# KevynUtopia/Frequency-Aware-Inverse-Consistent-OCTA-Super-Resolution

Hardware: AMD Instinct MI355X
Metric: train-step images/sec (G+D fwd+bwd) on 256x256 OCTA (higher is better)
Workload: dtype f32 (tensors and accumulators fp32; the convolutions' operands enter the matrix cores as f16x2 pairs: hi = f16(x 2^k), lo = f16(x 2^k - hi), k from the tensor's largest magnitude; 3 v_mfma_f32_32x32x16_f16 per product) on every map >= 24 wide with >= 16 channels; narrow maps, 1-channel stems / head

## Files before the change

### frequency-aware-inverse-consistent-octa-super-resolution_amd/csrc/igemm_bf16x3.hip

```cpp
#include "common.h"
#include "igemm_geom.h"
#include "pack_bodies.h"
#include "split16.h"
#include <cstdlib>
#include <cstdint>
#include <type_traits>

#ifndef SP_NCW8
#define SP_NCW8 0
#endif
#ifndef SP_MIN_W
#define SP_MIN_W 24
#endif
#ifndef SP_CDMA
#define SP_CDMA 0
#endif
#ifndef SP_SPLIT_BELOW
#define SP_SPLIT_BELOW 128
#endif
#ifndef SP_WIDE
#define SP_WIDE 1
#endif
#ifndef SP_PROD_FIRST
#define SP_PROD_FIRST 0
// ... 34 lines not shown

#ifndef SP_EPI_FAST
#define SP_EPI_FAST 1
#endif
#ifndef SP_ABLATE
#define SP_ABLATE 0
#endif

constexpr int SP_MT = 64;
static thread_local bool g_conv_residual_live = false;
constexpr int SP_NPI = 6;

__device__ __forceinline__ int reflect_idx_s(int i, int n) {
    i = i < 0 ? -i : i;
    return i >= n ? 2 * n - 2 - i : i;
}

__device__ __forceinline__ void ds_read_v8(bf16x8& dst, unsigned addr) { asm volatile("ds_read_b128 %0, %1" : "=v"(dst) : "v"(addr)); }

template <int I, int N, class F>
__device__ __forceinline__ void static_for_sp(F&& f) {
    if constexpr (I < N) {
        f(std::integral_constant<int, I>{});
        static_for_sp<I + 1, N>(f);
    }
}

template <int MI, int NI>
__device__ __forceinline__ void wait_all(bf16x8 (&a)[MI][2], bf16x8 (&b)[NI][2]) {
    if constexpr (MI == 2 && NI == 2)
        asm volatile("s_waitcnt lgkmcnt(0)" : "+v"(a[0][0]), "+v"(a[0][1]), "+v"(a[1][0]), "+v"(a[1][1]), "+v"(b[0][0]), "+v"(b[0][1]), "+v"(b[1][0]), "+v"(b[1][1]));
    else if constexpr (MI == 2 && NI == 1)
        asm volatile("s_waitcnt lgkmcnt(0)" : "+v"(a[0][0]), "+v"(a[0][1]), "+v"(a[1][0]), "+v"(a[1][1]), "+v"(b[0][0]), "+v"(b[0][1]));
    else if constexpr (MI == 1 && NI == 2)
        asm volatile("s_waitcnt lgkmcnt(0)" : "+v"(a[0][0]), "+v"(a[0][1]), "+v"(b[0][0]), "+v"(b[0][1]), "+v"(b[1][0]), "+v"(b[1][1]));
    else
        asm volatile("s_waitcnt lgkmcnt(0)" : "+v"(a[0][0]), "+v"(a[0][1]), "+v"(b[0][0]), "+v"(b[0][1]));
}

template <int MI, int NI>
__device__ __forceinline__ void wait_keep_next(bf16x8 (&a)[MI][2], bf16x8 (&b)[NI][2]) {
    if constexpr (MI == 2 && NI == 2)
        asm volatile("s_waitcnt lgkmcnt(8)" : "+v"(a[0][0]), "+v"(a[0][1]), "+v"(a[1][0]), "+v"(a[1][1]), "+v"(b[0][0]), "+v"(b[0][1]), "+v"(b[1][0]), "+v"(b[1][1]));
    else if constexpr (MI == 2 && NI == 1)
        asm volatile("s_waitcnt lgkmcnt(6)" : "+v"(a[0][0]), "+v"(a[0][1]), "+v"(a[1][0]), "+v"(a[1][1]), "+v"(b[0][0]), "+v"(b[0][1]));
    else if constexpr (MI == 1 && NI == 2)
        asm volatile("s_waitcnt lgkmcnt(6)" : "+v"(a[0][0]), "+v"(a[0][1]), "+v"(b[0][0]), "+v"(b[0][1]), "+v"(b[1][0]), "+v"(b[1][1]));
    else
        asm volatile("s_waitcnt lgkmcnt(4)" : "+v"(a[0][0]), "+v"(a[0][1]), "+v"(b[0][0]), "+v"(b[0][1]));
}

template <bool F16>
__global__ __launch_bounds__(256) void split_pack_kernel(const float* __restrict__ w, unsigned short* __restrict__ wp, const SplitGeom g) {
    split_pack_block<F16>(w, wp, g, blockIdx.x, gridDim.x);
}
__global__ __launch_bounds__(256) void split_absmax_kernel(const float* __restrict__ w, float* __restrict__ wp, const SplitGeom g) {
    __shared__ unsigned red[4];
    split_absmax_block(w, wp, g, (int)blockIdx.x, red);
}

template <int NI, int SI, bool QUAD, int NCW = 4, bool F16 = false>
__global__ __launch_bounds__(64 * (NCW + 4)) void igemm_bf16x3_kernel(const float* __restrict__ x, const __bf16* __restrict__ wp,
                                                           const float* __restrict__ bias, float* __restrict__ y, const SplitGeom g,
                                                           const int ksplit, const int wide, const unsigned* __restrict__ x_slot,
                                                           const unsigned* __restrict__ w_slot, const float* __restrict__ res) {
    constexpr int MI = 2, TH = NCW * NI, NT = 256, NPI = SP_NPI;
    extern __shared__ __attribute__((aligned(16))) char smem[];
    const int tid = threadIdx.x, lane = tid & 63, wave = tid >> 6;
    SPTRACE0(tid == 0, 8);
    const int l31 = lane & 31, lh = lane >> 5;
    const bool producer = (SP_PROD_FIRST && NCW == 4) ? wave < 4 : wave >= NCW;
    const int wn = NCW == 4 ? wave & 3 : (wave >= NCW ? wave - NCW : wave), stid = tid & 255;
    const int ph = blockIdx.z / ksplit, ks = blockIdx.z - ph * ksplit;
    const int GH = g.gh[ph], GW = g.gw[ph];
    const int tiles_x = (GW + 31) >> 5, tiles_y = (GH + TH - 1) / TH;
    const int tiles = tiles_x * tiles_y;
    const long total_tiles = (long)g.N * tiles;
    if ((long)blockIdx.x >= total_tiles) return;
#if SP_STAGGER
    for (int i = (int)((blockIdx.x + blockIdx.y + blockIdx.z) & 7); i > 0; --i) __builtin_amdgcn_s_sleep(SP_STAGGER);
#endif
    const int t0 = g.t0[ph], T = g.t0[ph + 1] - t0, TG = g.tg[ph];
    const int ntg = (T + TG - 1) / TG;
    const int PH = (TH - 1) * SI + g.span_y[ph] + 1, PW = 31 * SI + g.span_x[ph] + 1, PHW = PH * PW;
    const int ngroups = (g.C + 15) >> 4;
    const int gps = (ngroups + ksplit - 1) / ksplit;
    const int g0 = ks * gps;
    const int g1 = (g0 + gps) < ngroups ? (g0 + gps) : ngroups;
    if (g0 >= g1) return;
    const int m0 = blockIdx.y * SP_MT;
    const int IH = g.IH, IW = g.IW;
    const long chw = (long)IH * IW;
    const unsigned a_bytes = (unsigned)TG * 2048u;
    const unsigned p_bytes = (unsigned)(2 * PHW) * 16u;
    const unsigned A_base = 0, P_base = 4u * a_bytes, S_base = P_base + 4u * p_bytes;
    auto tile_coords = [&](long tl, int& n, int& ty, int& tx) {
        n = (int)((unsigned)tl / (unsigned)tiles);
        const int rt = (int)((unsigned)tl - (unsigned)n * (unsigned)tiles);
        ty = (int)((unsigned)rt / (unsigned)tiles_x);
        tx = rt - ty * tiles_x;
    };

    if (producer) {
        if constexpr (SP_PRIO != 0) __builtin_amdgcn_s_setprio(SP_PRIO);
        constexpr unsigned OOB = 0x80000000u;
        const unsigned cstep = 4u * (unsigned)chw;
        const float* xin = x;
        float sx = 1.f;
        constexpr int NSI = QUAD ? 2 : NPI;
        unsigned poff[NSI];
        float pv[NSI][8];
        constexpr int NQI = QUAD ? 2 : 1;
        unsigned qoff[NQI];
        f32x4s qv[NQI][8];
        const int qx0 = (-g.ox0[ph]) & 3;
        const bool cover = QUAD && !g.reflect;
        const int qs = cover && qx0 ? qx0 - 4 : qx0;
        const int nq = QUAD ? (cover ? (PW - qs + 3) >> 2 : (PW - qx0) >> 2) : 0;
        const int ns = cover ? 0 : PW - 4 * nq;
        const int nqi = 2 * PH * nq, nitems = 2 * PH * ns;
        int s_pos[NSI], q_pos[NQI];
        int s_slot[NSI], q_slot[NQI];
        {
            const float inv_ns = 1.0f / (float)(ns > 0 ? ns : 1), inv_nq = 1.0f / (float)(nq > 0 ? nq : 1);
#pragma unroll
            for (int i = 0; i < NSI; ++i) {
                const int it = stid + NT * i;
                s_pos[i] = -1;
                s_slot[i] = 0;
                if (it < nitems) {
                    const int h = it >= PH * ns ? 1 : 0;
                    const int r = it - h * PH * ns;
                    const int py = (int)(((float)r + 0.5f) * inv_ns);
                    const int sx = r - py * ns;
                    const int px = sx < qx0 ? sx : sx + 4 * nq;
                    s_pos[i] = py | ((px + 4) << 8) | (h << 16);
                    s_slot[i] = h * PHW + py * PW + px;
                }
            }
#pragma unroll
            for (int i = 0; i < NQI; ++i) {
                const int it = stid + NT * i;
                q_pos[i] = -1;
                q_slot[i] = 0;
                if (QUAD && it < nqi) {
                    const int h = it >= PH * nq ? 1 : 0;
                    const int r = it - h * PH * nq;
                    const int py = (int)(((float)r + 0.5f) * inv_nq);
                    const int px = qs + 4 * (r - py * nq);
                    q_pos[i] = py | ((px + 4) << 8) | (h << 16);
                    q_slot[i] = h * PHW + py * PW + px;
                }
            }
        }
        if constexpr ((SP_ABLATE & 2) != 0) {
            for (int i = 0; i < NSI; ++i)
                for (int j = 0; j < 8; ++j) pv[i][j] = (float)(tid + i + j);
            for (int i = 0; i < NQI; ++i)
                for (int j = 0; j < 8; ++j) qv[i][j] = f32x4s{(float)tid, (float)i, (float)j, 1.f};
        }
        auto compute_poff = [&](long tl) {
            int n, ty, tx;
            tile_coords(tl, n, ty, tx);
            const int y_base = ty * TH * SI + g.oy0[ph], x_base = tx * 32 * SI + g.ox0[ph];
            xin = x + (long)n * g.C * chw;
            auto off_of = [&](int pos) -> unsigned {
                if (pos < 0) return OOB;
                int iy = y_base + (pos & 0xff), ix = x_base + ((pos >> 8) & 0xff) - 4;
                if (g.reflect) {
                    iy = reflect_idx_s(iy, IH);
                    ix = reflect_idx_s(ix, IW);
                }
                if ((unsigned)iy < (unsigned)IH && (unsigned)ix < (unsigned)IW) return 4u * (unsigned)(8 * (pos >> 16) * (int)chw + iy * IW + ix);
                return OOB;
            };
#pragma unroll
            for (int i = 0; i < NSI; ++i) poff[i] = off_of(s_pos[i]);
#pragma unroll
            for (int i = 0; i < NQI; ++i) qoff[i] = off_of(q_pos[i]);
        };
        auto load_patch = [&](int grp) {
            if constexpr ((SP_ABLATE & 2) != 0) return;
            const long bytes = (long)(g.C - grp * 16) * chw * 4;
            const auto srd = __builtin_amdgcn_make_buffer_rsrc(const_cast<float*>(xin + (long)grp * 16 * chw), 0,
                                                               (int)(bytes < 0x7ffffff0L ? bytes : 0x7ffffff0L), 0x00020000);
            if constexpr (QUAD) {
#pragma unroll
                for (int i = 0; i < NQI; ++i)
                    if (NT * i < nqi) {
#pragma unroll
                        for (int j = 0; j < 8; ++j)
                            qv[i][j] = __builtin_bit_cast(f32x4s, __builtin_amdgcn_raw_buffer_load_b128(srd, qoff[i] + j * cstep, 0, 0));
                    }
            }
#pragma unroll
            for (int i = 0; i < NSI; ++i)
                if (NT * i < nitems) {
#pragma unroll
                    for (int j = 0; j < 8; ++j)
                        pv[i][j] = __builtin_bit_cast(float, __builtin_amdgcn_raw_buffer_load_b32(srd, poff[i] + j * cstep, 0, 0));
                }
        };
        auto store_patch = [&](int buf, auto&& hook) {
            if constexpr ((SP_ABLATE & 4) != 0) return;
            char* hi_p = smem + P_base + (buf * 2 + 0) * p_bytes;
            char* lo_p = smem + P_base + (buf * 2 + 1) * p_bytes;
            if constexpr (QUAD) {
#pragma unroll
                for (int i = 0; i < NQI; ++i) {
                    if (NT * i < nqi) {
                        const bool qok = q_pos[i] >= 0;
                        const int px0 = ((q_pos[i] >> 8) & 0xff) - 4;
#pragma unroll
                        for (int kp = 0; kp < 2; ++kp) {
                            unsigned hd[2][4], ld[2][4];
                            if constexpr (F16) {
#pragma unroll
                                for (int k = 0; k < 2; ++k) {
#pragma unroll
                                    for (int c2 = 0; c2 < 4; ++c2) {
                                        split_pair_scaled<true>(qv[i][2 * c2][2 * kp + k], qv[i][2 * c2 + 1][2 * kp + k], sx, hd[k][c2], ld[k][c2]);
                                        if (c2 & 1) hook();
                                    }
                                }
                            } else {
                            f32x2s lo[8];
#pragma unroll
                            for (int k = 0; k < 2; ++k)
#pragma unroll
                                for (int c2 = 0; c2 < 4; ++c2)
                                    hd[k][c2] = cvt_pair<F16>(qv[i][2 * c2][2 * kp + k], qv[i][2 * c2 + 1][2 * kp + k]);
                            hook();
#pragma unroll
                            for (int c = 0; c < 8; ++c) {
                                const unsigned d0 = hd[0][c >> 1], d1 = hd[1][c >> 1];
                                const f32x2s hf = {(c & 1) ? half_hi_f32<F16>(d0) : half_lo_f32<F16>(d0), (c & 1) ? half_hi_f32<F16>(d1) : half_lo_f32<F16>(d1)};
                                lo[c] = f32x2s{qv[i][c][2 * kp], qv[i][c][2 * kp + 1]} - hf;
                                if ((c & 3) == 3) hook();
                            }
#pragma unroll
                            for (int k = 0; k < 2; ++k)
#pragma unroll
                                for (int c2 = 0; c2 < 4; ++c2)
                                    ld[k][c2] = cvt_pair<F16>(lo[2 * c2][k], lo[2 * c2 + 1][k]);
                            }
#pragma unroll
                            for (int k = 0; k < 2; ++k) {
                                if (qok && (unsigned)(px0 + 2 * kp + k) < (unsigned)PW) {
                                    *reinterpret_cast<u32x4s*>(hi_p + (q_slot[i] + 2 * kp + k) * 16) = u32x4s{hd[k][0], hd[k][1], hd[k][2], hd[k][3]};
                                    *reinterpret_cast<u32x4s*>(lo_p + (q_slot[i] + 2 * kp + k) * 16) = u32x4s{ld[k][0], ld[k][1], ld[k][2], ld[k][3]};
                                }
                                hook();
                            }
                        }
                    }
                }
            }
#pragma unroll
            for (int i = 0; i < NSI; ++i) {
                if (s_pos[i] >= 0) {
                    u32x4s hv, lv;
#pragma unroll
                    for (int j = 0; j < 4; ++j) {
                        unsigned h, l;
                        split_pair_scaled<F16>(pv[i][2 * j], pv[i][2 * j + 1], sx, h, l);
                        hv[j] = h;
                        lv[j] = l;
                    }
                    *reinterpret_cast<u32x4s*>(hi_p + s_slot[i] * 16) = hv;
                    *reinterpret_cast<u32x4s*>(lo_p + s_slot[i] * 16) = lv;
                }
            }
        };
        const int wnu = __builtin_amdgcn_readfirstlane(wn);
        const char* const wbase = reinterpret_cast<const char*>(wp + g.pack_off[ph] + (long)m0 * 8);
        const long w_row = (long)g.Mpad * 16, w_plane = g.plane_stride * 2;
        const unsigned lane16 = (unsigned)lane * 16u;
        const char* d_src = wbase;
        char* d_dst = smem;
        int d_r = 0, d_rows = 0, d_rows2 = 0;
        auto begin_A = [&](int grp, int tgi, int abuf) {
            const int tb = tgi * TG;
            int nt = T - tb;
            nt = nt < TG ? nt : TG;
            d_rows = nt * 2;
            d_rows2 = ((SP_ABLATE & 1) || SP_CDMA) ? 0 : 2 * d_rows;
            d_r = wnu;
            d_src = wbase + ((long)grp * T + tb) * 2 * w_row;
            d_dst = smem + A_base + (abuf * 2) * a_bytes;
        };
        auto next_row = [&]() {
            if (d_r < d_rows2) {
                const int plane = d_r >= d_rows ? 1 : 0;
                const int rr = d_r - plane * d_rows;
                __builtin_amdgcn_global_load_lds((const __attribute__((address_space(1))) void*)(d_src + plane * w_plane + rr * w_row + lane16),
                                                 (__attribute__((address_space(3))) void*)(d_dst + plane * a_bytes + rr * 1024), 16, 0, 0);
                d_r += 4;
            }
            __builtin_amdgcn_sched_barrier(0);
        };
        auto rest_of_A = [&]() {
            while (d_r < d_rows2) next_row();
        };

        long tile_l = blockIdx.x;
        int grp_l = g0;
        bool valid_l = true;
        auto advance_l = [&]() {
            if (++grp_l >= g1) {
                grp_l = g0;
                tile_l += gridDim.x;
                valid_l = tile_l < total_tiles;
                if (valid_l) compute_poff(tile_l);
            }
        };
        int npl_full = 0;
        if constexpr ((SP_ABLATE & 2) == 0) {
            for (int i = 0; i < NQI; ++i) npl_full += (QUAD && NT * i < nqi) ? 8 : 0;
            for (int i = 0; i < NSI; ++i) npl_full += NT * i < nitems ? 8 : 0;
        }
        auto barrier_keep = [&](int n) {
            switch (n) {
                case 0: asm volatile("s_waitcnt vmcnt(0) lgkmcnt(0)\n\ts_barrier" ::: "memory"); break;
                case 8: asm volatile("s_waitcnt vmcnt(8) lgkmcnt(0)\n\ts_barrier" ::: "memory"); break;
                case 16: asm volatile("s_waitcnt vmcnt(16) lgkmcnt(0)\n\ts_barrier" ::: "memory"); break;
                case 24: asm volatile("s_waitcnt vmcnt(24) lgkmcnt(0)\n\ts_barrier" ::: "memory"); break;
                case 32: asm volatile("s_waitcnt vmcnt(32) lgkmcnt(0)\n\ts_barrier" ::: "memory"); break;
                case 40: asm volatile("s_waitcnt vmcnt(40) lgkmcnt(0)\n\ts_barrier" ::: "memory"); break;
                case 48: asm volatile("s_waitcnt vmcnt(48) lgkmcnt(0)\n\ts_barrier" ::: "memory"); break;
                default: asm volatile("s_waitcnt vmcnt(0) lgkmcnt(0)\n\ts_barrier" ::: "memory"); break;
            }
        };
        auto no_hook = [&]() {};

        SPTRACE0(tid == ((SP_PROD_FIRST && NCW == 4) ? 0 : 64 * NCW), 12);
        compute_poff(tile_l);
        load_patch(grp_l);
        SPTRACE0(tid == ((SP_PROD_FIRST && NCW == 4) ? 0 : 64 * NCW), 13);
        advance_l();
        begin_A(g0, 0, 0);
        if constexpr (SP_CDMA != 0) d_rows2 = (SP_ABLATE & 1) ? 0 : 2 * d_rows;
        rest_of_A();
        SPTRACE0(tid == ((SP_PROD_FIRST && NCW == 4) ? 0 : 64 * NCW), 14);
        if constexpr (F16) sx = f16x2_scale(absmax_read(x_slot));
        store_patch(0, no_hook);
        int in_flight = 0;
        if (valid_l) {
            load_patch(grp_l);
            advance_l();
        }
        SPTRACE0(tid == ((SP_PROD_FIRST && NCW == 4) ? 0 : 64 * NCW), 9);
        barrier_keep(0);
        SPTRACE0(tid == ((SP_PROD_FIRST && NCW == 4) ? 0 : 64 * NCW), 10);
        long tile = blockIdx.x;
        int slab = 0, pcount = 0;
        while (true) {
            const long next_tile = tile + gridDim.x;
            const bool has_next = next_tile < total_tiles;
            for (int grp = g0; grp < g1; ++grp, ++pcount) {
                const int pbuf = pcount & 1;
                const bool last_grp = grp + 1 >= g1;
                const bool more_patch = !last_grp || has_next;
                for (int tgi = 0; tgi < ntg; ++tgi, ++slab) {
                    const int abuf = slab & 1;
                    SPTRACE(tid == ((SP_PROD_FIRST && NCW == 4) ? 0 : 64 * NCW), 3072, slab, 0);
                    in_flight = 0;
                    const bool swap_patch = tgi == ntg - 1 && more_patch;
                    d_rows2 = 0;
                    if (tgi + 1 < ntg) begin_A(grp, tgi + 1, abuf ^ 1);
                    else if (!last_grp) begin_A(grp + 1, 0, abuf ^ 1);
                    else if (has_next) begin_A(g0, 0, abuf ^ 1);
                    if (swap_patch) store_patch(pbuf ^ 1, next_row);
                    SPTRACE(tid == ((SP_PROD_FIRST && NCW == 4) ? 0 : 64 * NCW), 1024, slab, 0);
                    rest_of_A();
                    SPTRACE(tid == ((SP_PROD_FIRST && NCW == 4) ? 0 : 64 * NCW), 1024, slab, 1);
                    if (swap_patch && valid_l) {
                        load_patch(grp_l);
                        advance_l();
                        in_flight = npl_full;
                    }
                    SPTRACE(tid == ((SP_PROD_FIRST && NCW == 4) ? 0 : 64 * NCW), 1024, slab, 2);
                    barrier_keep(in_flight);
                    SPTRACE(tid == ((SP_PROD_FIRST && NCW == 4) ? 0 : 64 * NCW), 1024, slab, 3);
                }
            }
            if (!has_next) break;
            tile = next_tile;
        }
        return;
    }

    int tapv = 0;
    if (lane < T) {
        const int tp = g.taps[t0 + lane];
        tapv = (tp & 0xff) * PW + ((tp >> 8) & 0xff);
    }
    f32x16 acc[MI][NI];
#pragma unroll
    for (int mi = 0; mi < MI; ++mi)
#pragma unroll
        for (int ni = 0; ni < NI; ++ni)
#pragma unroll
            for (int r = 0; r < 16; ++r) acc[mi][ni][r] = 0.f;
    const unsigned lds0 = (unsigned)(unsigned long)(__attribute__((address_space(3))) char*)smem;
    const unsigned a_lane = (unsigned)(lh * 64 + l31) * 16u;
    const unsigned b_lane = (unsigned)((lh * PH + (wn * NI) * SI) * PW + l31 * SI) * 16u;
    const unsigned b_row = (unsigned)(SI * PW) * 16u;

    const int wnu_c = __builtin_amdgcn_readfirstlane(wn);
    const char* const wbase_c = reinterpret_cast<const char*>(wp + g.pack_off[ph] + (long)m0 * 8);
    const long w_row_c = (long)g.Mpad * 16, w_plane_c = g.plane_stride * 2;
    const unsigned lane16_c = (unsigned)lane * 16u;
    const char* c_src = wbase_c;
    char* c_dst = smem;
    int c_r = 0, c_rows = 0, c_rows2 = 0;
    auto c_begin = [&](int grp, int tgi, int abuf) {
        const int tb2 = tgi * TG;
        int nt2 = T - tb2;
        nt2 = nt2 < TG ? nt2 : TG;
        c_rows = nt2 * 2;
        c_rows2 = 2 * c_rows;
        c_r = wnu_c;
        c_src = wbase_c + ((long)grp * T + tb2) * 2 * w_row_c;
        c_dst = smem + A_base + (abuf * 2) * a_bytes;
    };
    auto c_next_row = [&]() {
        if (c_r < c_rows2) {
            const int plane = c_r >= c_rows ? 1 : 0;
            const int rr = c_r - plane * c_rows;
            __builtin_amdgcn_global_load_lds((const __attribute__((address_space(1))) void*)(c_src + plane * w_plane_c + rr * w_row_c + lane16_c),
                                             (__attribute__((address_space(3))) void*)(c_dst + plane * a_bytes + rr * 1024), 16, 0, 0);
            c_r += 4;
        }
    };

    float inv = 1.f;
    if constexpr (F16) inv = f16x2_inv_scale(absmax_read(x_slot)) * f16x2_inv_scale(split_w_absmax(w_slot));
    long tile = blockIdx.x;
    asm volatile("s_barrier" ::: "memory");
    int slab = 0, pcount = 0;
    while (true) {
        const long next_tile = tile + gridDim.x;
        const bool has_next = next_tile < total_tiles;
        for (int grp = g0; grp < g1; ++grp, ++pcount) {
            const int pbuf = pcount & 1;
            for (int tgi = 0; tgi < ntg; ++tgi, ++slab) {
                const int abuf = slab & 1;
                const int tb = tgi * TG;
                int nt = T - tb;
                nt = nt < TG ? nt : TG;
                const unsigned Ah = lds0 + A_base + (abuf * 2 + 0) * a_bytes + a_lane, Al = Ah + a_bytes;
                const unsigned Ph = lds0 + P_base + (pbuf * 2 + 0) * p_bytes + b_lane, Pl = Ph + p_bytes;
                bf16x8 a0[MI][2], b0[NI][2], a1[MI][2], b1[NI][2];
                auto rd_all = [&](bf16x8 (&a)[MI][2], bf16x8 (&b)[NI][2], int tl) {
                    const unsigned ao = (unsigned)tl * 2048u;
                    const unsigned bo = 16u * (unsigned)__builtin_amdgcn_readlane(tapv, (tb + tl) & 63);
#pragma unroll
                    for (int mi = 0; mi < MI; ++mi) {
                        ds_read_v8(a[mi][0], Ah + ao + mi * 512u);
                        ds_read_v8(a[mi][1], Al + ao + mi * 512u);
                    }
#pragma unroll
                    for (int ni = 0; ni < NI; ++ni) {
                        ds_read_v8(b[ni][0], Ph + bo + ni * b_row);
                        ds_read_v8(b[ni][1], Pl + bo + ni * b_row);
                    }
                };
                auto step = [&](bf16x8 (&a)[MI][2], bf16x8 (&b)[NI][2], bf16x8 (&an)[MI][2], bf16x8 (&bn)[NI][2], int tl_next) {
                    const unsigned ao = (unsigned)tl_next * 2048u;
                    const unsigned bo = 16u * (unsigned)__builtin_amdgcn_readlane(tapv, (tb + tl_next) & 63);
                    wait_all<MI, NI>(a, b);
                    static_for_sp<0, 3 * MI * NI>([&](auto jc) {
                        constexpr int j = decltype(jc)::value;
                        constexpr int term = j / (MI * NI), t = j % (MI * NI), mi = t / NI, ni = t % NI;
                        if constexpr ((SP_ABLATE & 8) != 0) {
                            if constexpr (j == 0) acc[0][0][0] += (float)a[0][0][0] + (float)a[MI - 1][1][0] + (float)b[0][0][0] + (float)b[NI - 1][1][0];
                        } else {
                            mfma16<F16>(a[mi][term == 0 ? 1 : 0], b[ni][term == 1 ? 1 : 0], acc[mi][ni]);
                        }
                        if constexpr (j < 2 * MI) ds_read_v8(an[j / 2][j % 2], (j % 2 ? Al : Ah) + ao + (j / 2) * 512u);
                        else if constexpr (j < 2 * (MI + NI)) ds_read_v8(bn[(j - 2 * MI) / 2][(j - 2 * MI) % 2], ((j - 2 * MI) % 2 ? Pl : Ph) + bo + ((j - 2 * MI) / 2) * b_row);
                        __builtin_amdgcn_sched_barrier(0);
                    });
                };
                SPTRACE(tid == ((SP_PROD_FIRST && NCW == 4) ? 256 : 0), 2048, slab, 0);
                if constexpr (SP_CDMA != 0) {
                    c_rows2 = 0;
                    const bool last_grp_c = grp + 1 >= g1;
                    if (tgi + 1 < ntg) c_begin(grp, tgi + 1, abuf ^ 1);
                    else if (!last_grp_c) c_begin(grp + 1, 0, abuf ^ 1);
// ... 112 lines not shown
                        for (int rr = 0; rr < 16; ++rr) S[((rr & 3) + 8 * (rr >> 2) + 4 * lh) * 32 + l31] = acc[mi][ni][rr];
#pragma unroll
                        for (int i = 0; i < 4; ++i) {
                            f32x4s v = *reinterpret_cast<const f32x4s*>(S + (prow + 8 * i) * 32 + 4 * pq);
                            const int dm = mi * 32 + 8 * i;
                            if (ok && (full_m || m0 + prow + dm < g.M) && ((SP_ABLATE & 16) == 0 || v[0] == 123.456f)) {
                                if (res) v += *reinterpret_cast<const f32x4s*>(rimg + (o0 + (unsigned)dm * ohw));
                                *reinterpret_cast<f32x4s*>(yimg + (o0 + (unsigned)dm * ohw)) = v;
                            }
                        }
                    }
                }
            } else
#pragma unroll
            for (int ni = 0; ni < NI; ++ni) {
                const int ao = cty * TH + wn * NI + ni;
                if (ao < GH && bo < GW) {
                    const unsigned o0 = (unsigned)mrow0 * ohw + (unsigned)((ao * g.SO + g.py[ph]) * g.OW + (bo * g.SO + g.px[ph]));
                    if (SP_EPI_FAST && (SP_ABLATE & 16) == 0 && full_m) {
                        auto emit = [&](auto atomic_c, auto res_c) {
                            constexpr bool AT = decltype(atomic_c)::value, RS = decltype(res_c)::value;
#pragma unroll
                            for (int mi = 0; mi < MI; ++mi) {
                                float r[16];
                                if constexpr (RS) {
#pragma unroll
                                    for (int rr = 0; rr < 16; ++rr) r[rr] = rimg[o0 + (unsigned)(mi * 32 + (rr & 3) + 8 * (rr >> 2)) * ohw];
                                }
#pragma unroll
                                for (int rr = 0; rr < 16; ++rr) {
                                    float* const p = yimg + (o0 + (unsigned)(mi * 32 + (rr & 3) + 8 * (rr >> 2)) * ohw);
                                    float v = acc[mi][ni][rr];
                                    if constexpr (RS) v += r[rr];
                                    if constexpr (AT) atomicAdd(p, v);
                                    else *p = v;
                                }
                            }
                        };
                        const bool use_res = res && ks == 0;
                        if (ksplit > 1) {
                            if (use_res) emit(std::true_type{}, std::true_type{});
                            else emit(std::true_type{}, std::false_type{});
                        } else {
                            if (use_res) emit(std::false_type{}, std::true_type{});
                            else emit(std::false_type{}, std::false_type{});
                        }
                    } else
#pragma unroll
                    for (int mi = 0; mi < MI; ++mi) {
#pragma unroll
                        for (int rr = 0; rr < 16; ++rr) {
                            const int dm = mi * 32 + (rr & 3) + 8 * (rr >> 2);
                            if ((full_m || mrow0 + dm < g.M) && ((SP_ABLATE & 16) == 0 || acc[mi][ni][rr] == 123.456f)) {
                                float* const p = yimg + (o0 + (unsigned)dm * ohw);
                                const float rv = (res && ks == 0) ? rimg[o0 + (unsigned)dm * ohw] : 0.f;
                                if (ksplit > 1) atomicAdd(p, acc[mi][ni][rr] + rv);
                                else *p = acc[mi][ni][rr] + rv;
                            }
                        }
                    }
                }
            }
            SPTRACE(tid == ((SP_PROD_FIRST && NCW == 4) ? 256 : 0), 3584, slab, 2);
#pragma unroll
            for (int mi = 0; mi < MI; ++mi)
#pragma unroll
                for (int ni = 0; ni < NI; ++ni)
#pragma unroll
                    for (int r = 0; r < 16; ++r) acc[mi][ni][r] = 0.f;
            SPTRACE(tid == ((SP_PROD_FIRST && NCW == 4) ? 256 : 0), 3584, slab, 3);
        }
        if (!has_next) break;
        tile = next_tile;
    }
    SPTRACE0(tid == ((SP_PROD_FIRST && NCW == 4) ? 256 : 0), 11);
}

constexpr size_t SP_LDS_MAX = 156 * 1024;

static size_t sp_lds(const SplitGeom& g, int NI, int SI, bool staging = true, int ncw = 4) {
    const int TH = 4 * NI;
    size_t best = 0;
    for (int p = 0; p < g.nphase; ++p) {
        const int PH = (TH - 1) * SI + g.span_y[p] + 1, PW = 31 * SI + g.span_x[p] + 1;
        const size_t b = 4 * (size_t)g.tg[p] * 2048 + 4 * (size_t)(2 * PH * PW) * 16 + (staging ? 4096 * (size_t)ncw : 0) + 2048;
        best = b > best ? b : best;
    }
    return best;
}

static bool sp_fits(const SplitGeom& g, int NI, int SI) {
    const int TH = 4 * NI;
    for (int p = 0; p < g.nphase; ++p) {
        const int PH = (TH - 1) * SI + g.span_y[p] + 1, PW = 31 * SI + g.span_x[p] + 1;
        if (2 * PH * PW > 256 * SP_NPI) return false;
    }
    return sp_lds(g, NI, SI, false) <= SP_LDS_MAX;
}

int split_geom_from(const IgemmGeom& f, SplitGeom& g, int f16, bool narrow) {
    g = SplitGeom{};
    g.f16 = f16 ? 1 : 0;
    {
        const long a = (long)f.M * f.wsm, b = (long)f.C * f.wsc;
        g.w_elems = a > b ? a : b;
    }
    g.N = f.N; g.C = f.C; g.IH = f.IH; g.IW = f.IW; g.M = f.M; g.OH = f.OH; g.OW = f.OW; g.SI = f.SI; g.SO = f.SO;
    g.nphase = f.nphase; g.reflect = f.reflect; g.act = f.act; g.slope = f.slope; g.wsm = f.wsm; g.wsc = f.wsc;
    if (g.C < 16 || (g.SI != 1 && g.SI != 2)) return 0;
    for (int p = 0; p < 4; ++p) { g.py[p] = f.ph_py[p]; g.px[p] = f.ph_px[p]; g.gh[p] = f.ph_gh[p]; g.gw[p] = f.ph_gw[p]; }
    for (int p = 0; p < 5; ++p) g.t0[p] = f.ph_t0[p];
    g.Mpad = (g.M + 63) / 64 * 64;
    long off = 0;
    const int ngroups = (g.C + 15) / 16;
    for (int p = 0; p < g.nphase; ++p) {
        const int T = g.t0[p + 1] - g.t0[p];
        if (T == 0 || (!narrow && g.gw[p] < SP_MIN_W)) return 0;
        int oy0 = 1 << 30, ox0 = 1 << 30, oy1 = -(1 << 30), ox1 = -(1 << 30);
        for (int t = g.t0[p]; t < g.t0[p + 1]; ++t) {
            const int oy = (f.taps[t] & 0xff) - 64, ox = ((f.taps[t] >> 8) & 0xff) - 64;
            oy0 = oy < oy0 ? oy : oy0; ox0 = ox < ox0 ? ox : ox0;
            oy1 = oy > oy1 ? oy : oy1; ox1 = ox > ox1 ? ox : ox1;
        }
        g.oy0[p] = oy0; g.ox0[p] = ox0; g.span_y[p] = oy1 - oy0; g.span_x[p] = ox1 - ox0;
        int tg = T;
        if (T > 9) {
            tg = 8;
            for (int cand = 9; cand >= 5; --cand)
                if (T % cand == 0) { tg = cand; break; }
        }
        g.tg[p] = tg;
        g.pack_off[p] = off;
        off += (long)ngroups * T * 16 * g.Mpad;
        for (int t = g.t0[p]; t < g.t0[p + 1]; ++t) {
            const int oy = (f.taps[t] & 0xff) - 64, ox = ((f.taps[t] >> 8) & 0xff) - 64, wi = f.taps[t] >> 16;
            g.taps[t] = (oy - oy0) | ((ox - ox0) << 8) | (wi << 16);
        }
    }
    for (int p = g.nphase; p < 5; ++p) g.pack_off[p] = off;
    g.plane_stride = (off + 7) & ~7L;
    if (narrow) return 1;
    if (!sp_fits(g, 2, g.SI) && !sp_fits(g, 1, g.SI)) return 0;
    return 1;
}

#ifndef SP_QUAD
#define SP_QUAD 1
#endif
static bool sp_quad_ok(const SplitGeom& g, int NI, const float* x) {
    if (!SP_QUAD || (g.IW & 3) || (reinterpret_cast<uintptr_t>(x) & 15)) return false;
    const int TH = 4 * NI;
    for (int p = 0; p < g.nphase; ++p) {
        const int PH = (TH - 1) * g.SI + g.span_y[p] + 1, PW = 31 * g.SI + g.span_x[p] + 1;
        const int qx0 = (-g.ox0[p]) & 3;
        const bool cover = !g.reflect;
        const int qs = cover && qx0 ? qx0 - 4 : qx0;
        const int nq = cover ? (PW - qs + 3) >> 2 : (PW - qx0) >> 2, ns = cover ? 0 : PW - 4 * nq;
        if (nq < 1 || 2 * PH * nq > 512 || 2 * PH * ns > 512 || PH > 255 || PW > 240) return false;
        if (g.reflect) {
            const int tiles_x = (g.gw[p] + 31) / 32;
            if (g.ox0[p] + qx0 < 0 || (tiles_x - 1) * 32 * g.SI + g.ox0[p] + qx0 + 4 * nq > g.IW) return false;
        }
    }
    return true;
}

long split_pack_floats(const SplitGeom& g) { return g.plane_stride + 512; }
// ... 160 lines not shown
```

### frequency-aware-inverse-consistent-octa-super-resolution_amd/csrc/wgrad_x3.hip

```cpp
#include <type_traits>

#include "common.h"
#include "split16.h"
#include "igemm_geom.h"

namespace faoctasr {

typedef float f32x16 __attribute__((ext_vector_type(16)));
typedef float f32x4 __attribute__((ext_vector_type(4)));
typedef __bf16 bf16x8 __attribute__((ext_vector_type(8)));
typedef __bf16 bf16x4 __attribute__((ext_vector_type(4)));
typedef unsigned u32x2 __attribute__((ext_vector_type(2)));
typedef unsigned u32x4 __attribute__((ext_vector_type(4)));

struct WgX3Geom {
    int N, C, H, W, M;
    long wsm, wsc;
    int tiles_x, tiles_y, tiles_per_block;
    int gx, gy, slices;
    long dw_elems;
};

constexpr int X3_DLD = 72;
constexpr int X3_PROWS = 4, X3_PCOLS = 40;
// ... 172 lines not shown
            auto rd = [&](auto sc, auto jc) {
                constexpr int s = decltype(sc)::value, j = decltype(jc)::value;
                constexpr int kb = s / 3, kh = s % 3, set = s & 1;
                if constexpr (j < 12) {
                    constexpr int kw = j >> 2, which = j & 3;
                    constexpr unsigned imm = (unsigned)(((kb >> 1) + kh) * X3_PCOLS + 16 * (kb & 1) + kw + 3) * 64u;
                    if constexpr (which == 0) x3_read_tr<imm>(bh[set][kw][0], b_addr);
                    else if constexpr (which == 1) x3_read_tr<imm + 4 * 64>(bh[set][kw][1], b_addr);
                    else if constexpr (which == 2) x3_read_tr<imm + X3_XPLANE>(bl[set][kw][0], b_addr);
                    else x3_read_tr<imm + 4 * 64 + X3_XPLANE>(bl[set][kw][1], b_addr);
                } else if constexpr (kh == 0) {
                    constexpr unsigned a_imm = 2u * (unsigned)((kb >> 1) * 32 + 16 * (kb & 1));
                    if constexpr (j == 12) x3_read_128<a_imm>(a_hi[kb & 1], a_addr);
                    else x3_read_128<a_imm + X3_DPLANE>(a_lo[kb & 1], a_addr);
                }
            };
            x3_static_for<0, 14>([&](auto jc) { rd(std::integral_constant<int, 0>{}, jc); });
            x3_static_for<0, 12>([&](auto sc) {
                constexpr int s = decltype(sc)::value;
                constexpr int kb = s / 3, kh = s % 3, set = s & 1, ab = kb & 1;
                x3_wait_set(a_hi[ab], a_lo[ab], bh[set], bl[set]);
                __builtin_amdgcn_sched_barrier(0);
                x3_static_for<0, 9>([&](auto mc) {
                    constexpr int m = decltype(mc)::value, kw = m / 3, term = m % 3;
                    const bf16x8 b_hi = __builtin_shufflevector(bh[set][kw][0], bh[set][kw][1], 0, 1, 2, 3, 4, 5, 6, 7);
                    const bf16x8 b_lo = __builtin_shufflevector(bl[set][kw][0], bl[set][kw][1], 0, 1, 2, 3, 4, 5, 6, 7);
                    f32x16& d = acc[kh * 3 + kw];
                    if constexpr (term == 0) mfma16<F16>(a_lo[ab], b_hi, d);
                    else if constexpr (term == 1) mfma16<F16>(a_hi[ab], b_lo, d);
                    else mfma16<F16>(a_hi[ab], b_hi, d);
                    if constexpr (s + 1 < 12 && m < 7) {
                        rd(std::integral_constant<int, s + 1>{}, std::integral_constant<int, 2 * m>{});
                        rd(std::integral_constant<int, s + 1>{}, std::integral_constant<int, 2 * m + 1>{});
                    }
                    __builtin_amdgcn_sched_barrier(0);
                });
            });
        }
        asm volatile("s_waitcnt lgkmcnt(0)\n\ts_barrier" ::: "memory");
    }

    float* stage = reinterpret_cast<float*>(smem) + wave * 2304;
    const long col_base = (long)(c0 + cb * 32) * g.wsc;
    float inv = 1.f;
    if constexpr (F16) inv = f16x2_inv_scale(absmax_read(x_slot)) * f16x2_inv_scale(absmax_read(dy_slot));
#pragma unroll
    for (int j = 0; j < 4; ++j) {
#pragma unroll
        for (int t = 0; t < 9; ++t)
#pragma unroll
            for (int r = 0; r < 4; ++r) stage[((r + 4 * lh) * 32 + l31) * 9 + t] = F16 ? acc[t][4 * j + r] * inv : acc[t][4 * j + r];
        __builtin_amdgcn_fence(__ATOMIC_RELEASE, "wavefront");
        __builtin_amdgcn_wave_barrier();
        __builtin_amdgcn_fence(__ATOMIC_ACQUIRE, "wavefront");
        auto flush = [&](auto two_pass) {
            float* const out = decltype(two_pass)::value ? ws + (long)slice * g.dw_elems : dw;
#pragma unroll
            for (int i0 = 0; i0 < 36; i0 += 12) {
                float v[12];
#pragma unroll
                for (int i = 0; i < 12; ++i) v[i] = stage[lane + 64 * (i0 + i)];
#pragma unroll
                for (int i = 0; i < 12; ++i) {
                    const int e = lane + 64 * (i0 + i);
                    const int row = e / 288, col = e - row * 288;
                    const long o = (long)(m0 + mh * 32 + 8 * j + row) * g.wsm + col_base + col;
                    if constexpr (decltype(two_pass)::value) out[o] = v[i];
                    else atomicAdd(out + o, v[i]);
                }
            }
        };
        if (ws) flush(std::true_type{});
        else flush(std::false_type{});
        __builtin_amdgcn_fence(__ATOMIC_RELEASE, "wavefront");
        __builtin_amdgcn_wave_barrier();
        __builtin_amdgcn_fence(__ATOMIC_ACQUIRE, "wavefront");
    }
}

constexpr int X3R_PROWS = 2;
template <int S> struct X3R {
    static constexpr int PCOLS = S == 1 ? X3_PCOLS : 72;
    static constexpr int NCK = PCOLS / 4;
    static constexpr unsigned CB_BYTES = X3R_PROWS * PCOLS * 64;
    static constexpr unsigned XPLANE = 2 * CB_BYTES;
    static constexpr unsigned LDS = 2 * X3_DPLANE + 2 * XPLANE;
    static constexpr int NXI = (2 * 8 * X3R_PROWS * NCK + 255) / 256;
};

struct WgX3RowGeom {
    int N, C, H, W, OH, OW, M, KH, pad, reflect;
    long wsm, wsc;
    int tiles_x, tiles_y, tiles_per_block;
    int gx, gy, slices;
    long dw_elems;
};

template <int KW, int S, int PAD, bool F16>
__global__ __launch_bounds__(512) void wgrad_x3_row_kernel(const float* __restrict__ x, const float* __restrict__ dy, float* __restrict__ dw,
                                                           const WgX3RowGeom g, const unsigned* __restrict__ x_slot, const unsigned* __restrict__ dy_slot,
                                                           float* __restrict__ ws) {
    extern __shared__ __attribute__((aligned(16))) char smem[];
    const int tid = threadIdx.x, lane = tid & 63, wave = tid >> 6;
    const bool producer = wave >= 4;
    const int stid = tid & 255;
    const int l31 = lane & 31, lh = lane >> 5;
    const int mh = wave & 1, cb = (wave >> 1) & 1;

    const int per_slice = g.gx * g.gy * g.KH;
    const int bid = blockIdx.x;
    const int nfull = (g.slices / 8) * 8 * per_slice;
    int slice, inner;
    if (bid < nfull) {
        const int xcd = bid & 7, k = bid >> 3;
        inner = k % per_slice;
        slice = (k / per_slice) * 8 + xcd;
    } else {
        const int r = bid - nfull;
        inner = r % per_slice;
        slice = (g.slices / 8) * 8 + r / per_slice;
    }
    const int kh = inner % g.KH;
    const int rest = inner / g.KH;
    const int c0 = (rest % g.gx) * 64, m0 = (rest / g.gx) * 64;
    const long hw = (long)g.H * g.W, ohw = (long)g.OH * g.OW;
    typedef X3R<S> R;
    const long ntiles = (long)g.N * g.tiles_y * g.tiles_x;
    const long tile0 = (long)slice * g.tiles_per_block;
    long tile1 = tile0 + g.tiles_per_block;
    tile1 = tile1 < ntiles ? tile1 : ntiles;
    if (tile0 >= tile1) return;
    const int ntl = (int)(tile1 - tile0);

    const unsigned lds0 = (unsigned)(unsigned long)(__attribute__((address_space(3))) char*)smem;
    const unsigned d_lds0 = lds0, x_lds0 = lds0 + 2 * X3_DPLANE;

    if (producer) {
        float sx = 1.f, sd = 1.f;
        if constexpr (F16) { sx = f16x2_scale(absmax_read(x_slot)); sd = f16x2_scale(absmax_read(dy_slot)); }
        unsigned dg_off[2], dl_off[2];
#pragma unroll
        for (int i = 0; i < 2; ++i) {
            const int it = stid + 256 * i, m = it >> 3, ch = it & 7;
            dg_off[i] = 4u * (unsigned)(m * (int)ohw + (ch >> 2) * g.OW + (ch & 3) * 8);
            dl_off[i] = d_lds0 + 2u * (unsigned)(m * X3_DLD + (ch >> 2) * 32 + (ch & 3) * 8);
        }
        unsigned xc_off[R::NXI], xl_off[R::NXI];
        int x_row[R::NXI], x_ck[R::NXI];
#pragma unroll
        for (int i = 0; i < R::NXI; ++i) {
            const int it = stid + 256 * i;
            const int q8 = it & 7, rem = it >> 3;
            const int ck = rem % R::NCK, rc = rem / R::NCK;
            const int cbs = rc & 1, row = (rc >> 1) & 1;
            x_row[i] = rc < 4 ? row : -1;
            x_ck[i] = ck;
            xc_off[i] = 4u * (unsigned)((cbs * 8 + q8) * 4 * (int)hw);
            xl_off[i] = x_lds0 + (unsigned)cbs * R::CB_BYTES + (unsigned)(row * R::PCOLS + 4 * ck) * 64u + (unsigned)q8 * 8u;
        }
        int tn, ty, tx;
        {
            const long per_img = (long)g.tiles_y * g.tiles_x;
            tn = (int)(tile0 / per_img);
            const int r = (int)(tile0 - (long)tn * per_img);
            ty = r / g.tiles_x;
            tx = r - ty * g.tiles_x;
        }
        f32x4 dv[2][2], xv[R::NXI][4];
        int flip[R::NXI] = {};
        auto load_tile = [&]() {
            const int y0 = ty * 2, x0 = tx * 32;
            const float* dsrc = dy + ((long)tn * g.M + m0) * ohw + (long)y0 * g.OW + x0;
            const float* ximg = x + ((long)tn * g.C + c0) * hw;
            if (++tx == g.tiles_x) { tx = 0; if (++ty == g.tiles_y) { ty = 0; ++tn; } }
#pragma unroll
            for (int i = 0; i < 2; ++i) {
                const char* p = reinterpret_cast<const char*>(dsrc) + dg_off[i];
                dv[i][0] = *reinterpret_cast<const f32x4*>(p);
                dv[i][1] = *reinterpret_cast<const f32x4*>(p + 16);
            }
#pragma unroll
            for (int i = 0; i < R::NXI; ++i) {
                int iy = S * (y0 + x_row[i]) + kh - PAD, gx0 = S * x0 - 4 + 4 * x_ck[i];
                bool ok = x_row[i] >= 0;
                flip[i] = 0;
                if (g.reflect) {
                    iy = iy < 0 ? -iy : (iy >= g.H ? 2 * g.H - 2 - iy : iy);
                    if (gx0 < 0) { gx0 = 0; flip[i] = 1; }
                    else if (gx0 >= g.W) { gx0 = g.W - 4; flip[i] = 2; }
                } else {
                    ok = ok && (unsigned)iy < (unsigned)g.H && (unsigned)gx0 < (unsigned)g.W;
                }
#pragma unroll
                for (int c = 0; c < 4; ++c) {
                    xv[i][c] = f32x4{0.f, 0.f, 0.f, 0.f};
                    if (ok) xv[i][c] = *reinterpret_cast<const f32x4*>(reinterpret_cast<const char*>(ximg + (long)c * hw + (long)iy * g.W + gx0) + xc_off[i]);
                }
            }
        };
        auto store_tile = [&](int buf) {
            const unsigned bo = (unsigned)buf * R::LDS;
#pragma unroll
            for (int i = 0; i < 2; ++i) {
                unsigned h0, h1, h2, h3, l0, l1, l2, l3;
                split_pair_scaled<F16>(dv[i][0][0], dv[i][0][1], sd, h0, l0);
                split_pair_scaled<F16>(dv[i][0][2], dv[i][0][3], sd, h1, l1);
                split_pair_scaled<F16>(dv[i][1][0], dv[i][1][1], sd, h2, l2);
                split_pair_scaled<F16>(dv[i][1][2], dv[i][1][3], sd, h3, l3);
                const u32x4 hi = {h0, h1, h2, h3}, lo = {l0, l1, l2, l3};
                const unsigned da = dl_off[i] + bo;
                asm volatile("ds_write_b128 %0, %1" ::"v"(da), "v"(hi) : "memory");
                asm volatile("ds_write_b128 %0, %1 offset:%2" ::"v"(da), "v"(lo), "n"(X3_DPLANE) : "memory");
            }
#pragma unroll
            for (int i = 0; i < R::NXI; ++i) {
                if (x_row[i] < 0) continue;
                const unsigned xa = xl_off[i] + bo;
#pragma unroll
                for (int c = 0; c < 4; ++c) {
                    const f32x4 v = xv[i][c];
                    const f32x4 l = {v[0], v[3], v[2], v[1]}, r = {v[2], v[1], v[0], v[3]};
                    xv[i][c] = flip[i] == 1 ? l : (flip[i] == 2 ? r : v);
                }
#pragma unroll
                for (int px = 0; px < 4; ++px) {
                    unsigned h0, h1, l0, l1;
                    split_pair_scaled<F16>(xv[i][0][px], xv[i][1][px], sx, h0, l0);
                    split_pair_scaled<F16>(xv[i][2][px], xv[i][3][px], sx, h1, l1);
                    const u32x2 hi = {h0, h1}, lo = {l0, l1};
                    asm volatile("ds_write_b64 %0, %1 offset:%2" ::"v"(xa), "v"(hi), "n"(64 * px) : "memory");
                    asm volatile("ds_write_b64 %0, %1 offset:%2" ::"v"(xa), "v"(lo), "n"(64 * px + R::XPLANE) : "memory");
                }
            }
        };
        auto barrier = [&]() { asm volatile("s_waitcnt lgkmcnt(0)\n\ts_barrier" ::: "memory"); };
        load_tile();
        store_tile(0);
        if (ntl > 1) load_tile();
        barrier();
        for (int i = 0; i < ntl; ++i) {
            if (i + 1 < ntl) store_tile((i + 1) & 1);
            if (i + 2 < ntl) load_tile();
            barrier();
        }
        return;
    }

    const unsigned a_addr0 = d_lds0 + 2u * (unsigned)((mh * 32 + l31) * X3_DLD + 8 * lh);
    const int gi = lane & 15, q4 = gi >> 2, p4 = gi & 3, chh = (lane >> 4) & 1;
    const unsigned b_addr0 = x_lds0 + (unsigned)cb * R::CB_BYTES + (unsigned)(S * (8 * lh + q4)) * 64u + (unsigned)(chh * 4 + p4) * 8u;

    f32x16 acc[KW];
#pragma unroll
    for (int t = 0; t < KW; ++t)
#pragma unroll
        for (int r = 0; r < 16; ++r) acc[t][r] = 0.f;

    asm volatile("s_barrier" ::: "memory");
    for (int it = 0; it < ntl; ++it) {
        const unsigned a_addr = a_addr0 + (unsigned)(it & 1) * R::LDS, b_addr = b_addr0 + (unsigned)(it & 1) * R::LDS;
        x3_static_for<0, 4>([&](auto kc) {
            constexpr int kb = decltype(kc)::value;
            constexpr unsigned a_imm = 2u * (unsigned)((kb >> 1) * 32 + 16 * (kb & 1));
            bf16x8 a_hi, a_lo;
            asm volatile("ds_read_b128 %0, %1 offset:%2" : "=v"(a_hi) : "v"(a_addr), "n"(a_imm));
            asm volatile("ds_read_b128 %0, %1 offset:%2" : "=v"(a_lo) : "v"(a_addr), "n"(a_imm + X3_DPLANE));
            bf16x4 bh[KW][2], bl[KW][2];
            x3_static_for<0, KW>([&](auto wc) {
                constexpr int kw = decltype(wc)::value;
                constexpr unsigned imm = (unsigned)((kb >> 1) * R::PCOLS + S * 16 * (kb & 1) + kw + (4 - PAD)) * 64u;
                const unsigned ba = b_addr;
                bf16x4 h0, h1, l0, l1;
                asm volatile("ds_read_b64_tr_b16 %0, %1 offset:%2" : "=v"(h0) : "v"(ba), "n"(imm));
                asm volatile("ds_read_b64_tr_b16 %0, %1 offset:%2" : "=v"(h1) : "v"(ba), "n"(imm + S * 4 * 64));
                asm volatile("ds_read_b64_tr_b16 %0, %1 offset:%2" : "=v"(l0) : "v"(ba), "n"(imm + R::XPLANE));
                asm volatile("ds_read_b64_tr_b16 %0, %1 offset:%2" : "=v"(l1) : "v"(ba), "n"(imm + S * 4 * 64 + R::XPLANE));
                bh[kw][0] = h0; bh[kw][1] = h1; bl[kw][0] = l0; bl[kw][1] = l1;
            });
            asm volatile("s_waitcnt lgkmcnt(0)" : "+v"(a_hi), "+v"(a_lo));
            x3_static_for<0, KW>([&](auto wc) {
                constexpr int kw = decltype(wc)::value;
                bf16x4 h0 = bh[kw][0], h1 = bh[kw][1], l0 = bl[kw][0], l1 = bl[kw][1];
                asm volatile("" : "+v"(h0), "+v"(h1), "+v"(l0), "+v"(l1));
                bh[kw][0] = h0; bh[kw][1] = h1; bl[kw][0] = l0; bl[kw][1] = l1;
            });
            __builtin_amdgcn_sched_barrier(0);
#pragma unroll
            for (int kw = 0; kw < KW; ++kw) {
                const bf16x8 b_hi = __builtin_shufflevector(bh[kw][0], bh[kw][1], 0, 1, 2, 3, 4, 5, 6, 7);
                const bf16x8 b_lo = __builtin_shufflevector(bl[kw][0], bl[kw][1], 0, 1, 2, 3, 4, 5, 6, 7);
                f32x16& d = acc[kw];
                mfma16<F16>(a_lo, b_hi, d);
                mfma16<F16>(a_hi, b_lo, d);
                mfma16<F16>(a_hi, b_hi, d);
            }
        });
        asm volatile("s_waitcnt lgkmcnt(0)\n\ts_barrier" ::: "memory");
    }

    float* stage = reinterpret_cast<float*>(smem) + wave * (8 * 32 * KW);
    const long col_base = (long)(c0 + cb * 32) * g.wsc + (long)kh * KW;
    float inv = 1.f;
    if constexpr (F16) inv = f16x2_inv_scale(absmax_read(x_slot)) * f16x2_inv_scale(absmax_read(dy_slot));
#pragma unroll
    for (int j = 0; j < 4; ++j) {
#pragma unroll
        for (int t = 0; t < KW; ++t)
#pragma unroll
            for (int r = 0; r < 4; ++r) stage[((r + 4 * lh) * 32 + l31) * KW + t] = F16 ? acc[t][4 * j + r] * inv : acc[t][4 * j + r];
        __builtin_amdgcn_fence(__ATOMIC_RELEASE, "wavefront");
        __builtin_amdgcn_wave_barrier();
        __builtin_amdgcn_fence(__ATOMIC_ACQUIRE, "wavefront");
        auto flush = [&](auto two_pass) {
            float* const out = decltype(two_pass)::value ? ws + (long)slice * g.dw_elems : dw;
            constexpr int NE = (8 * 32 * KW + 63) / 64;
            static_assert(8 * 32 * KW % 64 == 0, "whole waves of elements");
            constexpr int NB = KW == 7 ? 7 : KW == 4 ? 8 : 6;
            static_assert(NE % NB == 0, "whole batches");
#pragma unroll
            for (int i0 = 0; i0 < NE; i0 += NB) {
                float v[NB];
#pragma unroll
                for (int i = 0; i < NB; ++i) v[i] = stage[lane + 64 * (i0 + i)];
#pragma unroll
                for (int i = 0; i < NB; ++i) {
                    const int e = lane + 64 * (i0 + i);
                    const int row = e / (32 * KW), rem = e - row * (32 * KW), ch = rem / KW, t = rem - ch * KW;
                    const long o = (long)(m0 + mh * 32 + 8 * j + row) * g.wsm + col_base + (long)ch * g.wsc + t;
                    if constexpr (decltype(two_pass)::value) out[o] = v[i];
                    else atomicAdd(out + o, v[i]);
                }
            }
        };
        if (ws) flush(std::true_type{});
        else flush(std::false_type{});
        __builtin_amdgcn_fence(__ATOMIC_RELEASE, "wavefront");
        __builtin_amdgcn_wave_barrier();
        __builtin_amdgcn_fence(__ATOMIC_ACQUIRE, "wavefront");
    }
}

__global__ __launch_bounds__(256) void wgrad_reduce_kernel(const float* __restrict__ ws, float* __restrict__ dw, long elems, int slices) {
    __shared__ f32x4 part[16][16];
    const int e = threadIdx.x & 15, grp = threadIdx.x >> 4;
    const long i = ((long)blockIdx.x * 16 + e) * 4;
    f32x4 s = {0.f, 0.f, 0.f, 0.f};
    if (i < elems) {
        const float* p = ws + i;
        int k = grp;
        for (; k + 48 < slices; k += 64) {
            const f32x4 a = *reinterpret_cast<const f32x4*>(p + (long)k * elems), b = *reinterpret_cast<const f32x4*>(p + (long)(k + 16) * elems);
            const f32x4 c = *reinterpret_cast<const f32x4*>(p + (long)(k + 32) * elems), d = *reinterpret_cast<const f32x4*>(p + (long)(k + 48) * elems);
            s += (a + b) + (c + d);
        }
        for (; k < slices; k += 16) s += *reinterpret_cast<const f32x4*>(p + (long)k * elems);
    }
    part[grp][e] = s;
    __syncthreads();
    if (grp == 0 && i < elems) {
// ... 98 lines not shown
```

Measured before the change: 136.8.

## Deinterleave stride-2 LDS patch columns into even/odd halves to avoid bank conflicts

For stride-2 convolutions (forward igemm and weight-gradient kernels), the LDS input patch is stored with even and odd columns in separate contiguous halves rather than interleaved. Consecutive lanes reading every other column then hit adjacent slots, which removes the strided LDS access pattern and its bank conflicts. All patch writers, tap offsets, lane bases and the LDS size calculation are updated to the new column mapping. It adds index arithmetic and a padded row width, and it only affects stride-2 layers.

```diff
diff --git a/frequency-aware-inverse-consistent-octa-super-resolution_amd/csrc/igemm_bf16x3.hip b/frequency-aware-inverse-consistent-octa-super-resolution_amd/csrc/igemm_bf16x3.hip
--- a/frequency-aware-inverse-consistent-octa-super-resolution_amd/csrc/igemm_bf16x3.hip
+++ b/frequency-aware-inverse-consistent-octa-super-resolution_amd/csrc/igemm_bf16x3.hip
@@ -140,7 +140,12 @@
 #endif
     const int t0 = g.t0[ph], T = g.t0[ph + 1] - t0, TG = g.tg[ph];
     const int ntg = (T + TG - 1) / TG;
-    const int PH = (TH - 1) * SI + g.span_y[ph] + 1, PW = 31 * SI + g.span_x[ph] + 1, PHW = PH * PW;
+    const int PH = (TH - 1) * SI + g.span_y[ph] + 1, PW = 31 * SI + g.span_x[ph] + 1;
+    const int PWh = (PW + 1) >> 1, PWS = SI == 2 ? 2 * PWh : PW, PHW = PH * PWS;
+    auto patch_col = [&](int px) {
+        if constexpr (SI == 2) return (px & 1) * PWh + (px >> 1);
+        else return px;
+    };
     const int ngroups = (g.C + 15) >> 4;
     const int gps = (ngroups + ksplit - 1) / ksplit;
     const int g0 = ks * gps;
@@ -193,7 +198,7 @@
                     const int sx = r - py * ns;
                     const int px = sx < qx0 ? sx : sx + 4 * nq;
                     s_pos[i] = py | ((px + 4) << 8) | (h << 16);
-                    s_slot[i] = h * PHW + py * PW + px;
+                    s_slot[i] = h * PHW + py * PWS + patch_col(px);
                 }
             }
 #pragma unroll
@@ -207,7 +212,7 @@
                     const int py = (int)(((float)r + 0.5f) * inv_nq);
                     const int px = qs + 4 * (r - py * nq);
                     q_pos[i] = py | ((px + 4) << 8) | (h << 16);
-                    q_slot[i] = h * PHW + py * PW + px;
+                    q_slot[i] = h * PHW + py * PWS + patch_col(px);
                 }
             }
         }
@@ -269,6 +274,7 @@
                     if (NT * i < nqi) {
                         const bool qok = q_pos[i] >= 0;
                         const int px0 = ((q_pos[i] >> 8) & 0xff) - 4;
+                        const int odd_d = SI == 2 ? ((px0 & 1) ? 1 - PWh : PWh) : 0;
 #pragma unroll
                         for (int kp = 0; kp < 2; ++kp) {
                             unsigned hd[2][4], ld[2][4];
@@ -305,8 +311,9 @@
 #pragma unroll
                             for (int k = 0; k < 2; ++k) {
                                 if (qok && (unsigned)(px0 + 2 * kp + k) < (unsigned)PW) {
-                                    *reinterpret_cast<u32x4s*>(hi_p + (q_slot[i] + 2 * kp + k) * 16) = u32x4s{hd[k][0], hd[k][1], hd[k][2], hd[k][3]};
-                                    *reinterpret_cast<u32x4s*>(lo_p + (q_slot[i] + 2 * kp + k) * 16) = u32x4s{ld[k][0], ld[k][1], ld[k][2], ld[k][3]};
+                                    const int slot = SI == 2 ? q_slot[i] + kp + (k ? odd_d : 0) : q_slot[i] + 2 * kp + k;
+                                    *reinterpret_cast<u32x4s*>(hi_p + slot * 16) = u32x4s{hd[k][0], hd[k][1], hd[k][2], hd[k][3]};
+                                    *reinterpret_cast<u32x4s*>(lo_p + slot * 16) = u32x4s{ld[k][0], ld[k][1], ld[k][2], ld[k][3]};
                                 }
                                 hook();
                             }
@@ -451,7 +458,7 @@
     int tapv = 0;
     if (lane < T) {
         const int tp = g.taps[t0 + lane];
-        tapv = (tp & 0xff) * PW + ((tp >> 8) & 0xff);
+        tapv = (tp & 0xff) * PWS + patch_col((tp >> 8) & 0xff);
     }
     f32x16 acc[MI][NI];
 #pragma unroll
@@ -462,8 +469,8 @@
             for (int r = 0; r < 16; ++r) acc[mi][ni][r] = 0.f;
     const unsigned lds0 = (unsigned)(unsigned long)(__attribute__((address_space(3))) char*)smem;
     const unsigned a_lane = (unsigned)(lh * 64 + l31) * 16u;
-    const unsigned b_lane = (unsigned)((lh * PH + (wn * NI) * SI) * PW + l31 * SI) * 16u;
-    const unsigned b_row = (unsigned)(SI * PW) * 16u;
+    const unsigned b_lane = (unsigned)((lh * PH + (wn * NI) * SI) * PWS + (SI == 2 ? l31 : l31 * SI)) * 16u;
+    const unsigned b_row = (unsigned)(SI * PWS) * 16u;
 
     const int wnu_c = __builtin_amdgcn_readfirstlane(wn);
     const char* const wbase_c = reinterpret_cast<const char*>(wp + g.pack_off[ph] + (long)m0 * 8);
@@ -742,7 +749,8 @@
     const int TH = 4 * NI;
     size_t best = 0;
     for (int p = 0; p < g.nphase; ++p) {
-        const int PH = (TH - 1) * SI + g.span_y[p] + 1, PW = 31 * SI + g.span_x[p] + 1;
+        const int PH = (TH - 1) * SI + g.span_y[p] + 1, PWr = 31 * SI + g.span_x[p] + 1;
+        const int PW = SI == 2 ? (PWr + 1) & ~1 : PWr;
         const size_t b = 4 * (size_t)g.tg[p] * 2048 + 4 * (size_t)(2 * PH * PW) * 16 + (staging ? 4096 * (size_t)ncw : 0) + 2048;
         best = b > best ? b : best;
     }
diff --git a/frequency-aware-inverse-consistent-octa-super-resolution_amd/csrc/wgrad_x3.hip b/frequency-aware-inverse-consistent-octa-super-resolution_amd/csrc/wgrad_x3.hip
--- a/frequency-aware-inverse-consistent-octa-super-resolution_amd/csrc/wgrad_x3.hip
+++ b/frequency-aware-inverse-consistent-octa-super-resolution_amd/csrc/wgrad_x3.hip
@@ -278,6 +278,7 @@
 template <int S> struct X3R {
     static constexpr int PCOLS = S == 1 ? X3_PCOLS : 72;
     static constexpr int NCK = PCOLS / 4;
+    static constexpr int col(int p) { return S == 1 ? p : (p & 1) * (PCOLS / 2) + (p >> 1); }
     static constexpr unsigned CB_BYTES = X3R_PROWS * PCOLS * 64;
     static constexpr unsigned XPLANE = 2 * CB_BYTES;
     static constexpr unsigned LDS = 2 * X3_DPLANE + 2 * XPLANE;
@@ -352,7 +353,7 @@
             x_row[i] = rc < 4 ? row : -1;
             x_ck[i] = ck;
             xc_off[i] = 4u * (unsigned)((cbs * 8 + q8) * 4 * (int)hw);
-            xl_off[i] = x_lds0 + (unsigned)cbs * R::CB_BYTES + (unsigned)(row * R::PCOLS + 4 * ck) * 64u + (unsigned)q8 * 8u;
+            xl_off[i] = x_lds0 + (unsigned)cbs * R::CB_BYTES + (unsigned)(row * R::PCOLS + R::col(4 * ck)) * 64u + (unsigned)q8 * 8u;
         }
         int tn, ty, tx;
         {
@@ -424,8 +425,8 @@
                     split_pair_scaled<F16>(xv[i][0][px], xv[i][1][px], sx, h0, l0);
                     split_pair_scaled<F16>(xv[i][2][px], xv[i][3][px], sx, h1, l1);
                     const u32x2 hi = {h0, h1}, lo = {l0, l1};
-                    asm volatile("ds_write_b64 %0, %1 offset:%2" ::"v"(xa), "v"(hi), "n"(64 * px) : "memory");
-                    asm volatile("ds_write_b64 %0, %1 offset:%2" ::"v"(xa), "v"(lo), "n"(64 * px + R::XPLANE) : "memory");
+                    asm volatile("ds_write_b64 %0, %1 offset:%2" ::"v"(xa), "v"(hi), "n"(64 * R::col(px)) : "memory");
+                    asm volatile("ds_write_b64 %0, %1 offset:%2" ::"v"(xa), "v"(lo), "n"(64 * R::col(px) + R::XPLANE) : "memory");
                 }
             }
         };
@@ -444,7 +445,7 @@
 
     const unsigned a_addr0 = d_lds0 + 2u * (unsigned)((mh * 32 + l31) * X3_DLD + 8 * lh);
     const int gi = lane & 15, q4 = gi >> 2, p4 = gi & 3, chh = (lane >> 4) & 1;
-    const unsigned b_addr0 = x_lds0 + (unsigned)cb * R::CB_BYTES + (unsigned)(S * (8 * lh + q4)) * 64u + (unsigned)(chh * 4 + p4) * 8u;
+    const unsigned b_addr0 = x_lds0 + (unsigned)cb * R::CB_BYTES + (unsigned)(8 * lh + q4) * 64u + (unsigned)(chh * 4 + p4) * 8u;
 
     f32x16 acc[KW];
 #pragma unroll
@@ -464,13 +465,13 @@
             bf16x4 bh[KW][2], bl[KW][2];
             x3_static_for<0, KW>([&](auto wc) {
                 constexpr int kw = decltype(wc)::value;
-                constexpr unsigned imm = (unsigned)((kb >> 1) * R::PCOLS + S * 16 * (kb & 1) + kw + (4 - PAD)) * 64u;
+                constexpr unsigned imm = (unsigned)((kb >> 1) * R::PCOLS + R::col(S * 16 * (kb & 1) + kw + (4 - PAD))) * 64u;
                 const unsigned ba = b_addr;
                 bf16x4 h0, h1, l0, l1;
                 asm volatile("ds_read_b64_tr_b16 %0, %1 offset:%2" : "=v"(h0) : "v"(ba), "n"(imm));
-                asm volatile("ds_read_b64_tr_b16 %0, %1 offset:%2" : "=v"(h1) : "v"(ba), "n"(imm + S * 4 * 64));
+                asm volatile("ds_read_b64_tr_b16 %0, %1 offset:%2" : "=v"(h1) : "v"(ba), "n"(imm + 4 * 64));
                 asm volatile("ds_read_b64_tr_b16 %0, %1 offset:%2" : "=v"(l0) : "v"(ba), "n"(imm + R::XPLANE));
-                asm volatile("ds_read_b64_tr_b16 %0, %1 offset:%2" : "=v"(l1) : "v"(ba), "n"(imm + S * 4 * 64 + R::XPLANE));
+                asm volatile("ds_read_b64_tr_b16 %0, %1 offset:%2" : "=v"(l1) : "v"(ba), "n"(imm + 4 * 64 + R::XPLANE));
                 bh[kw][0] = h0; bh[kw][1] = h1; bl[kw][0] = l0; bl[kw][1] = l1;
             });
             asm volatile("s_waitcnt lgkmcnt(0)" : "+v"(a_hi), "+v"(a_lo));
```

New measurement: 136.8, median of 4. Within noise of the previous version (+0.0%).
